# LIA-DiTella/DiffUDF

Hardware: AMD Instinct MI355X
Metric: train points/sec (SIREN fwd+∇x+Eikonal loss+bwd), 256×8 net, 100k pts (higher is better)
Workload: dtype f32

## Files before the change

### diffudf_amd/csrc/dudf_api.hip

```cpp
#include "dudf_internal.h"
#include <stdio.h>
#include <stdlib.h>
#include <string.h>
#include <vector>

namespace {
struct ProfRec { int slot; hipEvent_t e0, e1; };
bool g_prof_on = false;
std::vector<ProfRec> g_prof_recs;
std::vector<hipEvent_t> g_prof_pool;
hipEvent_t g_prof_open[PROF_NSLOTS];
const char* kProfNames[PROF_NSLOTS] = {"pack", "sweep_fwd", "sweep_rev", "sweep_adj_fwd", "sweep_adj_rev",
                                       "wgrad_hidden", "wgrad_small", "loss_fwd", "loss_bwd", "adam", "other"};
unsigned long long* g_prof_clk = nullptr;
hipEvent_t prof_event() {
    if (!g_prof_pool.empty()) { hipEvent_t e = g_prof_pool.back(); g_prof_pool.pop_back(); return e; }
    hipEvent_t e; (void)hipEventCreate(&e); return e;
}
}

namespace { int g_products[PROF_NSLOTS] = {0}; }
void dudf_note_products(int slot, int products) { if (slot >= 0 && slot < PROF_NSLOTS) g_products[slot] = products; }

unsigned long long* dudf_prof_clk(int slot) { return (g_prof_on && g_prof_clk) ? g_prof_clk + 2 * slot : nullptr; }
// ... 758 lines not shown
}

int dudf_get_option(const char* name, int* value) {
    if (!name || !value) return DUDF_E_BADMODE;
    for (int i = 0; i < OPT_COUNT; ++i)
        if (strcmp(name, kOpts[i].name) == 0) { *value = g_opt[i]; return 0; }
    return DUDF_E_BADMODE;
}

int dudf_reset_options(void) {
    for (int i = 0; i < OPT_COUNT; ++i) g_opt[i] = kOpts[i].def;
    return 0;
}

int dudf_set_wgrad_max_workgroups(int n) { return dudf_set_option("wgrad_max_workgroups", n); }

int dudf_abi_version(void) { return DUDF_ABI_VERSION; }

int dudf_profile_dump(char* buf, size_t buflen) {
    double tot[PROF_NSLOTS] = {0};
    long cnt[PROF_NSLOTS] = {0};
    for (auto& r : g_prof_recs) {
        float ms = 0.f;
        if (hipEventSynchronize(r.e1) == hipSuccess && hipEventElapsedTime(&ms, r.e0, r.e1) == hipSuccess) {
            tot[r.slot] += ms; cnt[r.slot] += 1;
        }
        g_prof_pool.push_back(r.e0); g_prof_pool.push_back(r.e1);
    }
    g_prof_recs.clear();
    size_t off = 0;
    for (int i = 0; i < PROF_NSLOTS; ++i) {
        if (!cnt[i]) continue;
        int w = snprintf(buf + off, off < buflen ? buflen - off : 0, "%s %ld %.6f\n", kProfNames[i], cnt[i], tot[i]);
        if (w < 0 || off + (size_t)w >= buflen) return DUDF_E_WORKSPACE;
        off += (size_t)w;
    }
    if (off < buflen) buf[off] = 0;
    return 0;
}

int dudf_debug_read_stash(const dudf_net_cfg* cfg, int which, int layer, int channel, int64_t n, int64_t n_hess,
                          float* out, void* workspace, size_t workspace_bytes, void* stream) {
    Ctx c;
    int rc = open_ctx(cfg, n, n_hess, workspace, workspace_bytes, stream, &c);
    if (rc) return rc;
    if (layer < 0 || layer >= c.lo.L || channel < 0 || channel > 3) return DUDF_E_BADCFG;
    const DudfLayout& lo = c.lo;
    const int64_t offs[8] = {lo.ws_S, lo.ws_C, lo.ws_Q, lo.ws_E, lo.ws_A, lo.ws_Z, lo.ws_R, lo.ws_ZS};
    if (which < 0 || which > 7) return DUDF_E_BADMODE;
    const bool sqaz = which == 0 || which == 2 || which == 4 || which == 5;
    const int b24 = which == 7 ? 0 : which == 1 ? ((lo.p24 & 4) ? 2 : 0) : sqaz ? ((lo.p24 & 1) ? 3 : 0) : ((lo.p24 & 2) ? 1 : 0);
    const int fxi = which == 0 ? 0 : which == 2 ? 1 : which == 4 ? 2 : 3;
    return dudf_launch_read_stash(lo, c.ws + offs[which], layer, channel, out, c.st, which == 1, b24,
                                  b24 == 3 ? c.ws + lo.ws_fx[fxi] : nullptr);
}

int dudf_debug_stash_layout(const dudf_net_cfg* cfg, int64_t n, int64_t n_hess, int64_t* out) {
    DudfLayout lo;
    int rc = dudf_make_layout(cfg, n, n_hess, &lo);
    if (rc) return rc;
    if (!out) return DUDF_E_BADCFG;
    const int64_t offs[8] = {lo.ws_S, lo.ws_C, lo.ws_Q, lo.ws_E, lo.ws_A, lo.ws_Z, lo.ws_R, lo.ws_ZS};
    for (int i = 0; i < 8; ++i) out[i] = offs[i] * (int64_t)sizeof(float);
    out[8] = lo.np * 16;
    out[9] = lo.stash_layer * (int64_t)sizeof(float);
    return 0;
}

int dudf_debug_kernel_choice(const dudf_net_cfg* cfg, int64_t n, int64_t n_hess, int which, int flags, char* name, size_t name_len) {
    DudfLayout lo;
    int rc = dudf_make_layout(cfg, n, n_hess, &lo, (flags & 16) != 0);
    if (rc) return rc;
    if (!name || name_len == 0) return DUDF_E_BADCFG;
    name[0] = 0;
    SweepChoice c;
    if (which == DUDF_CHOICE_WGRAD) {
        c = dudf_choose_wgrad(WgradRequest{lo.H, lo.L, lo.p24 & 1, lo.np}, dudf_options());
    } else {
        const SweepRequest r = {which & 15, lo.H, lo.L, flags & 1, (flags >> 1) & 1, (flags >> 2) & 1, (flags >> 3) & 1, split_mask(), lo.p24,
                                lo.ws_ebound != lo.ws_amax, lo.ws_zbound != lo.ws_amax};
        c = (which & DUDF_CHOICE_PAIR) ? dudf_choose_pair(r, dudf_options()) : dudf_choose_sweep(r, dudf_options());
    }
    if (c.status == 0 && dudf_choice_name(c, name, name_len) >= (int)name_len) return DUDF_E_WORKSPACE;
    return c.status;
}

int dudf_stash_mode(const dudf_net_cfg* cfg, int64_t n, int64_t n_hess) {
    DudfLayout lo;
    if (dudf_make_layout(cfg, n, n_hess, &lo)) return -1;
    return lo.p24;
}

}
```

### diffudf_amd/csrc/dudf_variants.h

```cpp
#pragma once
#include <stddef.h>
#include <stdint.h>
#include <stdio.h>
#include <utility>
#include "../../include/dudf_hip.h"

enum { SWEEP_FWD = 0, SWEEP_REV = 1, SWEEP_ADJ_FWD = 2, SWEEP_ADJ_REV = 3,
       SWEEP_FWD_H = 4, SWEEP_REV_H = 5, SWEEP_ADJ_FWD_H = 6, SWEEP_ADJ_REV_H = 7,
       SWEEP_FWD_J = 8 };

struct DudfOptions {
    int deterministic, split, split_quads, sweep_family, stash, wgrad_family, wgrad_tr, pair_launch, wgrad_max_workgroups, wgrad_buffers;
};
inline int dudf_split_mask(const DudfOptions& o) { return o.split ? (15 | (o.split_quads ? 32 : 0)) : 0; }

struct DudfVariant { int sw, fl, p24; };
constexpr DudfVariant kF32Variants[] = {{0, 3, 0}, {1, 1, 0}, {1, 0, 0}, {2, 0, 0}, {3, 1, 0}, {3, 0, 0},
                                        {4, 1, 0}, {5, 1, 0}, {5, 0, 0}, {6, 0, 0}, {7, 0, 0}, {8, 0, 0}};
constexpr DudfVariant kSweepVariants[] = {{0, 3, 1}, {0, 2, 0}, {0, 0, 0}, {1, 1, 1}, {1, 0, 0}, {2, 0, 1}, {3, 1, 1}, {3, 0, 1},
                                          {4, 1, 1}, {4, 0, 0}, {5, 1, 1}, {5, 0, 0}, {6, 0, 1}, {7, 0, 1}, {8, 0, 0}};
constexpr DudfVariant kWideVariants[] = {{0, 3, 1}, {0, 1, 0}, {1, 1, 1}, {1, 0, 0}, {2, 0, 1}, {3, 1, 1}, {3, 0, 1},
                                         {4, 1, 1}, {5, 1, 1}, {5, 0, 0}, {6, 0, 1}, {7, 0, 1}, {8, 0, 0}};
constexpr DudfVariant kPairVariants[] = {{0, 3, 1}, {1, 1, 1}, {2, 0, 1}, {3, 1, 1}};
constexpr int dudf_pair_flq(int sw) { return sw <= SWEEP_REV ? 1 : 0; }
// ... 104 lines not shown
    const bool h16 = which <= SWEEP_ADJ_REV ? ((r.split >> which) & 1) != 0 : (r.split & 32) != 0;
    int fl = fl_of(r);
    if (which == SWEEP_FWD) fl = r.store_c ? 3 : 1;
    if (which == SWEEP_FWD_H) fl = 1;
    const size_t lds16 = 3 * dudf_wide_chunk_bytes(2) + kAmaxBytes, lds = 3 * dudf_wide_chunk_bytes(3) + kAmaxBytes;
    if (r.p24) {
        const bool train_variant = which == SWEEP_FWD ? (r.store_s && r.store_c) : which == SWEEP_FWD_H ? r.store_s != 0
                                 : (which == SWEEP_REV || which == SWEEP_REV_H) ? r.train != 0 : which != SWEEP_FWD_J;
        if (r.p24 != 6 || !h16 || !train_variant) return dudf_no_choice(DUDF_E_UNSUPPORTED);
        return sweep_choice(r, DUDF_FAM_W16R, which, fl, 3, lds16, lds16);
    }
    return h16 ? sweep_choice(r, DUDF_FAM_W16, which, fl, 3, lds16, lds16) : sweep_choice(r, DUDF_FAM_W, which, fl, 6, lds, lds);
}
}

inline bool dudf_sweep_bf16_supported(int which, int H, int L) {
    return (H == 512 || H == 256 || H == 128) && L >= 2 && which >= SWEEP_FWD && which <= SWEEP_FWD_J;
}

inline SweepChoice dudf_choose_sweep(SweepRequest r, const DudfOptions& o) {
    if (r.which < SWEEP_FWD || r.which > SWEEP_FWD_J) return dudf_no_choice(DUDF_E_BADMODE);
    if (o.sweep_family && dudf_sweep_bf16_supported(r.which, r.H, r.L)) {
        const SweepChoice c = r.H == 512 ? dudf_detail::choose_w(r) : dudf_detail::choose_b(r);
        if (r.which >= SWEEP_FWD_H || c.status != DUDF_E_UNSUPPORTED) return c;
    }
    if (r.which <= SWEEP_ADJ_REV && r.p24) return dudf_no_choice(DUDF_E_UNSUPPORTED);
    if (r.which == SWEEP_FWD) r.store_s = r.store_c = 1;
    if (r.which == SWEEP_FWD_H) r.store_s = 1;
    if (!(r.H == 32 || r.H == 64 || r.H == 128 || r.H == 256 || r.H == 512)) return dudf_no_choice(DUDF_E_BADCFG);
    const int fl = r.which == SWEEP_FWD ? 3 : dudf_detail::fl_of(r);
    const size_t lds = 2 * 32 * (size_t)(r.H + 4) * sizeof(float);
    return dudf_detail::sweep_choice(r, DUDF_FAM_F32, r.which, fl, 1, lds, lds);
}

inline SweepChoice dudf_choose_pair(const SweepRequest& r, const DudfOptions& o) {
    const int base = r.which;
    const SweepChoice no = dudf_no_choice(DUDF_E_UNSUPPORTED);
    if (!o.sweep_family || !o.pair_launch || r.H != 256 || base < SWEEP_FWD || base > SWEEP_ADJ_REV) return no;
    if (!((r.split >> base) & 1) || r.L < 2 || r.L > kMaxLdsBiasLayers) return no;
    if (base == SWEEP_FWD && !(r.store_s && r.store_c)) return no;
    if (base == SWEEP_REV && !r.train) return no;
    if (base == SWEEP_ADJ_REV && !(r.have_e && r.ebound && ((r.split >> SWEEP_ADJ_FWD) & 1))) return no;
    const size_t w3 = 3 * dudf_chunk_bytes(256, 2), bias = base == SWEEP_FWD ? dudf_bias_bytes(r.L, 256) : 0;
    const size_t lds_p = w3 + (base == SWEEP_FWD ? bias : kAmaxBytes) + kOctBytes;
    const bool q16 = (r.split & 32) && r.zbound && r.ebound;
    const size_t lds_q = q16 ? w3 + bias + kAmaxBytes : 3 * dudf_chunk_bytes(256, 3) + kAmaxBytes;
    if (r.p24 && !(q16 && (r.p24 == 6 || r.p24 == 7))) return no;
    SweepChoice c = dudf_detail::sweep_choice(r, DUDF_FAM_PAIR, base, base == SWEEP_ADJ_FWD ? 0 : base == SWEEP_FWD ? 3 : 1, 3,
                                              lds_q > lds_p ? lds_q : lds_p, kLdsCu);
    c.swq = base + 4; c.flq = dudf_pair_flq(base); c.spq = q16; c.p24 = r.p24; c.no_pk = 1;
    return c;
}

struct WgradRequest { int H, L, p24; int64_t np; };
inline SweepChoice dudf_choose_wgrad(const WgradRequest& r, const DudfOptions& o) {
    const int H = r.H == 512 ? 256 : r.H, ntz = (r.H / H) * (r.H / H);
    auto pick = [&](int family, int var, int products, size_t lds) {
        SweepChoice c = {};
        c.family = family; c.H = H; c.fl = var; c.products = products; c.lds = c.lds_max = lds; c.p24 = family == DUDF_FAM_WG_F16P24;
        c.no_pk = family >= DUDF_FAM_WG_BF16P;
        return c;
    };
    if (!(H == 32 || H == 64 || H == 128 || H == 256)) return dudf_no_choice(DUDF_E_BADCFG);
    if (r.p24 && (o.wgrad_family != 0 || H != 256)) return dudf_no_choice(DUDF_E_UNSUPPORTED);
    if (o.wgrad_family == 1) return pick(DUDF_FAM_WG_F32, 0, 1, 4 * (size_t)(H / 4) * 33 * 4 * sizeof(float));
    const size_t lds_wave = (size_t)4 * 2 * (H / 4) * 16 * 4 * sizeof(float);
    if (H != 256 || o.wgrad_family == 2 || (int64_t)(r.H / 4) * r.np * 16 >= (1ll << 32)) return pick(DUDF_FAM_WG_BF16, 0, 6, lds_wave);
    const bool f16 = o.split && r.L <= kMaxAmaxLayers;
    const size_t lds_t = (size_t)(2 * 2 * 16 * 576);
    if (r.p24) {
        if (!(f16 && ntz == 1)) return dudf_no_choice(DUDF_E_UNSUPPORTED);
        return o.wgrad_buffers == 4 ? pick(DUDF_FAM_WG_F16P24, 25, 3, 4 * lds_t + 512) : pick(DUDF_FAM_WG_F16P24, 9, 3, 3 * lds_t + 512);
    }
    if (o.wgrad_tr && f16 && ntz == 1 && !o.deterministic) return pick(DUDF_FAM_WG_F16TR, 9, 3, 3 * lds_t + 512);
    const size_t lds_piece = (size_t)2 * (H / 32) * 2 * (32 * 16 + 16);
    if (f16) {
        SweepChoice c = pick(DUDF_FAM_WG_F16P, 9, 3, 3 * 2 * lds_piece + 512);
        c.remap = ntz == 4 && !o.deterministic;
        return c;
    }
    return pick(DUDF_FAM_WG_BF16P, 9, 6, 3 * 3 * lds_piece + 512);
}

inline int dudf_stash_p24_enabled(int H, int L, const DudfOptions& o) {
    int want = o.stash & 7;
    if (want != 0 && want != 6 && want != 7) want = 6;
    if (!(o.sweep_family && o.split && (dudf_split_mask(o) & 47) == 47)) want = 0;
    if (o.wgrad_family != 0) want &= 6;
    if (H == 256 && L >= 2 && L <= 32) return want;
    if (H == 512 && L >= 2) return want & 6;
    return 0;
}

inline int dudf_choice_name(const SweepChoice& c, char* buf, size_t n) {
    const char* np = c.no_pk ? "_np" : "";
    switch (c.family) {
        case DUDF_FAM_F32: return snprintf(buf, n, "sweep_kernel<%d,%d,%d>", c.H, c.sw, c.fl);
        case DUDF_FAM_BF16: return snprintf(buf, n, "sweep_bf16%s_kernel<%d,%d,%d>", np, c.H, c.sw, c.fl);
        case DUDF_FAM_F16:
            return snprintf(buf, n, "sweep_f16%s_kernel<%d,%d,%d>", np, c.H, c.sw, c.fl);
        case DUDF_FAM_F16R: return snprintf(buf, n, "sweep_f16r%s_kernel<%d,%d,%d>", np, c.H, c.sw, c.fl);
        case DUDF_FAM_F16P: return snprintf(buf, n, "sweep_f16p%s_kernel<%d,%d,%d>", np, c.H, c.sw, c.fl);
        case DUDF_FAM_W: return snprintf(buf, n, "sweep_w_kernel<%d,%d>", c.sw, c.fl);
        case DUDF_FAM_W16: return snprintf(buf, n, "sweep_w16_kernel<%d,%d>", c.sw, c.fl);
        case DUDF_FAM_W16R: return snprintf(buf, n, "sweep_w16r_kernel<%d,%d>", c.sw, c.fl);
        case DUDF_FAM_PAIR: return snprintf(buf, n, "sweep_pair_kernel<256,%d,%d,%d,%d,%d,%d>", c.swq, c.flq, c.sw, c.fl, c.spq, c.p24);
        case DUDF_FAM_WG_F32: return snprintf(buf, n, "wgrad_hidden_kernel<%d>", c.H);
        case DUDF_FAM_WG_BF16: return snprintf(buf, n, "wgrad_hidden_bf16_kernel<%d>", c.H);
        case DUDF_FAM_WG_BF16P: return snprintf(buf, n, "wgrad_hidden_bf16p_kernel<%d,%d>", c.H, c.fl);
        case DUDF_FAM_WG_F16P: return snprintf(buf, n, "wgrad_hidden_f16p_kernel<%d,%d>", c.H, c.fl);
        case DUDF_FAM_WG_F16TR: return snprintf(buf, n, "wgrad_hidden_f16tr_kernel<%d,%d>", c.H, c.fl);
        case DUDF_FAM_WG_F16P24: return snprintf(buf, n, "wgrad_hidden_f16p24_kernel<%d,%d>", c.H, c.fl);
        default: return snprintf(buf, n, "?");
    }
}
```

### diffudf_amd/csrc/dudf_wgrad.hip

```cpp
#include "dudf_internal.h"
#include <stdlib.h>
#include <string.h>
#include <type_traits>

namespace {

template <int H> struct WG;
template <> struct WG<256> { static constexpr int WO = 4, WI = 2, MT = 2, NTL = 4; };
template <> struct WG<128> { static constexpr int WO = 4, WI = 2, MT = 1, NTL = 2; };
template <> struct WG<64>  { static constexpr int WO = 2, WI = 2, MT = 1, NTL = 1; };
template <> struct WG<32>  { static constexpr int WO = 1, WI = 1, MT = 1, NTL = 1; };

constexpr int KT = 32;
constexpr int KTP = 33;

struct WgradArgs {
    const float *Q, *A, *Z, *S;
    int64_t ncol_h;
    float* dtheta;
    int64_t np, stash_layer, off_hid, hid_stride;
    int steps_total;
    int L;
    int have_g;
    int j0, nj;
    int Hs;
    int remap_nsplit;
    unsigned long long* clk;
    const unsigned* amax;
    int p24;
    const float *fxS, *fxQ, *fxA, *fxZ;
};

__device__ __forceinline__ f32x16 mfma32(float a, float b, f32x16 c) {
    return __builtin_amdgcn_mfma_f32_32x32x2f32(a, b, c, 0, 0, 0);
}

template <int H>
__device__ __forceinline__ void wgrad_hidden_body(const WgradArgs& a) {
    using W = WG<H>;
    constexpr int NTHR = 64 * W::WO * W::WI;
    constexpr int FQ = H / 4;
    constexpr int TILE = FQ * KTP * 4;
    constexpr int F4 = FQ * KT;
    constexpr int NLD = (F4 + NTHR - 1) / NTHR;
    extern __shared__ __attribute__((aligned(16))) float lds[];

    const int tid = threadIdx.x, lane = tid & 63, wave = tid >> 6;
    const int wo = wave / W::WI, wi = wave % W::WI;
    const int l32 = lane & 31, hh = lane >> 5;
    const int j = blockIdx.x + a.j0;
    const int nsplit = gridDim.y;
    const int s0 = (int)((int64_t)a.steps_total * blockIdx.y / nsplit);
    const int s1 = (int)((int64_t)a.steps_total * (blockIdx.y + 1) / nsplit);
    const int tz = a.Hs / H;
    const int o_off = (blockIdx.z / tz) * H, i_off = (blockIdx.z % tz) * H;
    const int64_t xrow = (int64_t)(o_off / 4) * a.np * 4, yrow = (int64_t)(i_off / 4) * a.np * 4;

    f32x16 acc[W::MT][W::NTL];
    float bsum[W::MT];
#pragma unroll
    for (int m = 0; m < W::MT; ++m) {
#pragma unroll
        for (int n = 0; n < W::NTL; ++n)
#pragma unroll
            for (int e = 0; e < 16; ++e) acc[m][n][e] = 0.f;
        bsum[m] = 0.f;
    }

    const int64_t lstride = a.stash_layer;
    const float* X0 = a.Q + (int64_t)(j + 1) * lstride + xrow;
    const float* X1 = a.Z + (int64_t)(j + 1) * lstride + xrow;
    const float* Y0 = a.A + (int64_t)j * lstride + yrow;
    const float* Y1 = a.S + (int64_t)j * lstride + yrow;

    f32x4 rx[NLD], ry[NLD];
    auto issue = [&](int pair, int step) {
#pragma unroll
        for (int u = 0; u < NLD; ++u) {
            const int f = tid + NTHR * u;
            if (F4 % NTHR == 0 || f < F4) {
                const int fq = f / KT, pt = f % KT;
                const int64_t off = ((int64_t)fq * a.np + (int64_t)step * KT + pt) * 4;
                rx[u] = *reinterpret_cast<const f32x4*>((pair ? X1 : X0) + off);
                ry[u] = *reinterpret_cast<const f32x4*>((pair ? Y1 : Y0) + off);
            }
        }
    };
    auto commit = [&](float* buf) {
#pragma unroll
        for (int u = 0; u < NLD; ++u) {
            const int f = tid + NTHR * u;
            if (F4 % NTHR == 0 || f < F4) {
                const int fq = f / KT, pt = f % KT;
                *reinterpret_cast<f32x4*>(buf + (fq * KTP + pt) * 4) = rx[u];
                *reinterpret_cast<f32x4*>(buf + TILE + (fq * KTP + pt) * 4) = ry[u];
            }
        }
    };

    const int npair = a.have_g ? 2 : 1;
    const int nit = npair * (s1 - s0);
    auto pair_of = [&](int it) { return a.have_g ? (it & 1) : 1; };
    auto step_of = [&](int it) { return s0 + (a.have_g ? (it >> 1) : it); };
    if (nit > 0) {
        issue(pair_of(0), step_of(0));
        commit(lds);
    }
    __syncthreads();
    for (int it = 0; it < nit; ++it) {
        const float* buf = lds + (it & 1) * 2 * TILE;
        if (it + 1 < nit) issue(pair_of(it + 1), step_of(it + 1));
        const float bflag = (pair_of(it) == 1 && wi == 0 && i_off == 0) ? 1.f : 0.f;
        const bool hstage = (int64_t)step_of(it) * KT < a.ncol_h;
        const float f_even = hstage ? (hh == 0 ? bflag : 0.f) : bflag;
// ... 610 lines not shown
        }
        DUDF_WSTAMP(4);
        if constexpr (HOT) {
            if constexpr (!(DBG & 1)) wait_raw(r, std::integral_constant<int, 2 * kSetLoads>{});
            DUDF_WSTAMP(6);
            if constexpr (!(DBG & 8)) split_store(it + 2, r, BW);
            DUDF_WSTAMP(8);
            if constexpr (!(DBG & 1)) load_raw(it + 5, r);
            publish(flag0 + 4u * (unsigned)wave, (unsigned)it + 3u);
        } else if (it + 2 < nit) {
            split_store(it + 2, r, BW);
            if (it + 5 < nit) load_raw_plain(it + 5, r);
            publish(flag0 + 4u * (unsigned)wave, (unsigned)it + 3u);
        }
        DUDF_WSTAMP(10);
        DUDF_WSTAMP(11);
    };
    int it = 0;
    const int nhot = nit >= 8 ? ((nit - 5) / 3) * 3 : 0;
    auto drain = [&]() {
        asm volatile("s_waitcnt vmcnt(0)" : "+v"(R0.g0), "+v"(R0.g1), "+v"(R0.g2), "+v"(R0.g3), "+v"(R1.g0), "+v"(R1.g1),
                     "+v"(R1.g2), "+v"(R1.g3), "+v"(R2.g0), "+v"(R2.g1), "+v"(R2.g2), "+v"(R2.g3));
        if constexpr (P24 == 1) asm volatile("" : "+v"(R0.sc), "+v"(R1.sc), "+v"(R2.sc));
    };
    drain();
    using B0 = std::integral_constant<int, 0>; using B1 = std::integral_constant<int, 1>; using B2 = std::integral_constant<int, 2>;
    for (; it < nhot; it += 3) {
        stage(it, R2, std::true_type{}, B0{});
        stage(it + 1, R0, std::true_type{}, B1{});
        stage(it + 2, R1, std::true_type{}, B2{});
    }
    drain();
    for (; it < nit; it += 3) {
        stage(it, R2, std::false_type{}, B0{});
        if (it + 1 < nit) stage(it + 1, R0, std::false_type{}, B1{});
        if (it + 2 < nit) stage(it + 2, R1, std::false_type{}, B2{});
    }
#if DUDF_WGRAD_DBG & 32
    if (bx == 3 && by == 10 && lane == 0)
        for (int i = 0; i < 12; ++i) g_wstamp[wave][i] = wst[i];
#endif

    float* dW = a.dtheta + a.off_hid + (int64_t)j * a.hid_stride + (int64_t)o_off * a.Hs + i_off;
    float* dB = a.dtheta + a.off_hid + (int64_t)j * a.hid_stride + (int64_t)a.Hs * a.Hs + o_off;
    if (nit > 0) {
        const int l32 = lane & 31, hh = lane >> 5;
#pragma unroll
        for (int m = 0; m < W::MT; ++m)
#pragma unroll
            for (int e = 0; e < 16; ++e) {
                const int o = (wo * W::MT + m) * 32 + (e & 3) + 8 * (e >> 2) + 4 * hh;
#pragma unroll
                for (int n = 0; n < W::NTL; ++n) {
                    const int i = (wi * W::NTL + n) * 32 + l32;
#if DUDF_WGRAD_DBG & 64
                    asm volatile("" :: "v"(acc[m][n][e]));
#else
                    atomicAdd(dW + (int64_t)o * a.Hs + i, SP != 0 ? acc[m][n][e] * inv_p : acc[m][n][e]);
#endif
                }
            }
        if (p_oper == 0 && i_off == 0) {
            if constexpr (P24 != 0) {
                const float bun = P24 == 1 ? 1.0f / sc1 : 1.0f;
                auto red = [&](float v, int f) {
                    v += __shfl_xor(v, 1); v += __shfl_xor(v, 2); v += __shfl_xor(v, 4); v += __shfl_xor(v, 8);
                    if (p_li == 0) atomicAdd(dB + f, v * bun);
                };
                const f32x4 bs[4] = {bacc, bacc1, bacc2, bacc3};
#pragma unroll
                for (int t = 0; t < 4; ++t)
#pragma unroll
                    for (int e = 0; e < 4; ++e) red(bs[t][e], 16 * (4 * pw + t) + 4 * p_q + e);
            } else {
            auto red = [&](float v, int f) {
                v += __shfl_xor(v, 1);
                v += __shfl_xor(v, 2);
                if (p_cg == 0) atomicAdd(dB + 4 * p_fq + f, v);
            };
            red(bacc.x, 0); red(bacc.y, 1); red(bacc.z, 2); red(bacc.w, 3);
            }
        }
    }
    if (clk_on && tid == 0) {
        a.clk[0] = __builtin_amdgcn_s_memtime() - clk_t0;
        a.clk[1] = __builtin_amdgcn_s_memrealtime() - clk_r0;
    }
}
template <int VAR> constexpr int wg_buffers() { static_assert(VAR == 9 || VAR == 25, "VAR 9: three image buffers, 25: four"); return VAR == 25 ? 4 : 3; }
template <int H, int VAR>
__global__ __launch_bounds__(64 * WG<H>::WO * WG<H>::WI) DUDF_NO_PK void wgrad_hidden_bf16p_kernel(WgradArgs a) {
    wgrad_hidden_bf16p_body<H, wg_buffers<VAR>()>(a);
}
template <int H, int VAR>
__global__ __launch_bounds__(64 * WG<H>::WO * WG<H>::WI) DUDF_NO_PK void wgrad_hidden_f16p_kernel(WgradArgs a) {
    wgrad_hidden_bf16p_body<H, wg_buffers<VAR>(), 1>(a);
}
template <int H, int VAR>
__global__ __launch_bounds__(64 * WG<H>::WO * WG<H>::WI) DUDF_NO_PK void wgrad_hidden_f16tr_kernel(WgradArgs a) {
    wgrad_hidden_bf16p_body<H, wg_buffers<VAR>(), 1, 2>(a);
}
template <int H, int VAR>
__global__ __launch_bounds__(64 * WG<H>::WO * WG<H>::WI) DUDF_NO_PK void wgrad_hidden_f16p24_kernel(WgradArgs a) {
    wgrad_hidden_bf16p_body<H, wg_buffers<VAR>(), 1, 1>(a);
}

#ifndef DUDF_WGSMALL_P24_PTS
#define DUDF_WGSMALL_P24_PTS 4096
#endif
struct WgradSmallArgs {
    const float *Q, *A, *Z, *S;
    const float *x4, *gbar, *ybar;
    float* dtheta;
    int64_t np, ncols, stash_layer, off_wo, off_bo;
    int H, L, have_g;
    int pts_per_block;
    float rho;
    const float *fxS, *fxQ, *fxA, *fxZ;
};

__device__ __forceinline__ float wave_sum(float v) {
#pragma unroll
    for (int o = 32; o > 0; o >>= 1) v += __shfl_xor(v, o);
    return v;
}

__device__ __forceinline__ void wgrad_small_body(const WgradSmallArgs& a) {
    const int lane = threadIdx.x & 63, wave = threadIdx.x >> 6;
    const int FQ = a.H / 4;
    const int64_t p0 = (int64_t)blockIdx.x * a.pts_per_block;
    const int64_t p1 = (p0 + a.pts_per_block < a.ncols) ? p0 + a.pts_per_block : a.ncols;
    const float* Q0 = a.Q;
    const float* Z0 = a.Z;
    const float* AL = a.A + (int64_t)(a.L - 1) * a.stash_layer;
    const float* SL = a.S + (int64_t)(a.L - 1) * a.stash_layer;
    const int fq_per = (FQ + gridDim.y - 1) / gridDim.y;
    const int fq_lo = blockIdx.y * fq_per, fq_hi = (fq_lo + fq_per < FQ) ? fq_lo + fq_per : FQ;
    for (int fq = fq_lo + wave; fq < fq_hi; fq += 4) {
        float w1[4][4], wo[4];
#pragma unroll
        for (int c = 0; c < 4; ++c) { wo[c] = 0.f; w1[c][0] = w1[c][1] = w1[c][2] = w1[c][3] = 0.f; }
#pragma unroll 4
        for (int64_t p = p0 + lane; p < p1; p += 64) {
            const int64_t off = ((int64_t)fq * a.np + p) * 4;
            const f32x4 z = __builtin_nontemporal_load(reinterpret_cast<const f32x4*>(Z0 + off));
            const f32x4 sl = __builtin_nontemporal_load(reinterpret_cast<const f32x4*>(SL + off));
            const f32x4 xv = *reinterpret_cast<const f32x4*>(a.x4 + p * 4);
            const float yb = a.ybar[p];
            f32x4 qv = {0, 0, 0, 0}, al = {0, 0, 0, 0}, gb = {0, 0, 0, 0};
            if (a.have_g) {
                qv = __builtin_nontemporal_load(reinterpret_cast<const f32x4*>(Q0 + off));
                al = __builtin_nontemporal_load(reinterpret_cast<const f32x4*>(AL + off));
                gb = *reinterpret_cast<const f32x4*>(a.gbar + p * 4);
            }
#pragma unroll
            for (int c = 0; c < 4; ++c) {
#pragma unroll
                for (int d = 0; d < 4; ++d) w1[c][d] += qv[c] * gb[d] + z[c] * xv[d];
                wo[c] += al[c] * xv[3] + yb * sl[c];
            }
        }
#pragma unroll
        for (int c = 0; c < 4; ++c) {
            const int f = 4 * fq + c;
#pragma unroll
            for (int d = 0; d < 4; ++d) {
                const float v = wave_sum(w1[c][d]);
                if (lane == 0) atomicAdd(d < 3 ? a.dtheta + f * 3 + d : a.dtheta + 3 * a.H + f, a.rho * v);
            }
            const float vo = wave_sum(wo[c]);
            if (lane == 0) atomicAdd(a.dtheta + a.off_wo + f, vo);
        }
    }
    if (wave == 0 && blockIdx.y == 0) {
        float s = 0.f;
        for (int64_t p = p0 + lane; p < p1; p += 64) s += a.ybar[p];
        s = wave_sum(s);
        if (lane == 0) atomicAdd(a.dtheta + a.off_bo, s);
    }
}
__global__ __launch_bounds__(256) DUDF_NO_PK void wgrad_small_kernel(WgradSmallArgs a) { wgrad_small_body(a); }

__device__ __forceinline__ f32x4 small_unpack24(const unsigned* g, const float sc) {
    typedef unsigned u3_t __attribute__((ext_vector_type(3)));
    const u3_t d = __builtin_nontemporal_load(reinterpret_cast<const u3_t*>(g));
    const unsigned d0 = d.x, d1 = d.y, d2 = d.z;
    const unsigned m = 0x00ffffffu, two = 0x40000000u;
    const unsigned y = __builtin_amdgcn_perm(d1, d0, 0x0c0c0703u);
    const unsigned t3 = __builtin_amdgcn_perm(d2, y, 0x0c070100u) | two;
    const float m3 = -3.0f * sc;
    return f32x4{__builtin_fmaf(__uint_as_float((d0 & m) | two), sc, m3), __builtin_fmaf(__uint_as_float((d1 & m) | two), sc, m3),
                 __builtin_fmaf(__uint_as_float((d2 & m) | two), sc, m3), __builtin_fmaf(__uint_as_float(t3), sc, m3)};
}
__global__ __launch_bounds__(256) DUDF_NO_PK void wgrad_small_p24_kernel(WgradSmallArgs a) {
    const int lane = threadIdx.x & 63, wave = threadIdx.x >> 6;
    const int q = lane >> 4, li = lane & 15, T = blockIdx.y;
    const int64_t ng = a.np >> 4;
    const int64_t g0 = (int64_t)blockIdx.x * (a.pts_per_block >> 4);
    const int64_t gend = (a.ncols + 15) >> 4;
    const int64_t g1 = g0 + (a.pts_per_block >> 4) < gend ? g0 + (a.pts_per_block >> 4) : gend;
    const int64_t lbytes = a.stash_layer * 3;
    auto tile = [&](const float* arr, int layer) { return reinterpret_cast<const char*>(arr) + (int64_t)layer * lbytes + (int64_t)T * ng * 768 + lane * 12; };
    const char* Q0 = tile(a.Q, 0); const char* Z0 = tile(a.Z, 0);
    const char* AL = tile(a.A, a.L - 1); const char* SL = tile(a.S, a.L - 1);
    float w1[4][4], wo[4];
#pragma unroll
    for (int c = 0; c < 4; ++c) { wo[c] = 0.f; w1[c][0] = w1[c][1] = w1[c][2] = w1[c][3] = 0.f; }
    float sy = 0.f;
    const int nwave = (int)(blockDim.x >> 6);
#pragma unroll 4
    for (int64_t g = g0 + wave; g < g1; g += nwave) {
        const int64_t p = g * 16 + li;
        const f32x4 z = small_unpack24(reinterpret_cast<const unsigned*>(Z0 + g * 768), a.fxZ[p]);
        const f32x4 sl = small_unpack24(reinterpret_cast<const unsigned*>(SL + g * 768), a.fxS[(int64_t)(a.L - 1) * a.np + p]);
        const f32x4 xv = *reinterpret_cast<const f32x4*>(a.x4 + p * 4);
        const float yb = a.ybar[p];
        f32x4 qv = {0, 0, 0, 0}, al = {0, 0, 0, 0}, gb = {0, 0, 0, 0};
        if (a.have_g) {
            qv = small_unpack24(reinterpret_cast<const unsigned*>(Q0 + g * 768), a.fxQ[p]);
            al = small_unpack24(reinterpret_cast<const unsigned*>(AL + g * 768), a.fxA[(int64_t)(a.L - 1) * a.np + p]);
            gb = *reinterpret_cast<const f32x4*>(a.gbar + p * 4);
        }
        sy += yb;
#pragma unroll
        for (int c = 0; c < 4; ++c) {
#pragma unroll
            for (int d = 0; d < 4; ++d) w1[c][d] += qv[c] * gb[d] + z[c] * xv[d];
            wo[c] += al[c] * xv[3] + yb * sl[c];
        }
    }
    auto sum16 = [](float v) { v += __shfl_xor(v, 1); v += __shfl_xor(v, 2); v += __shfl_xor(v, 4); v += __shfl_xor(v, 8); return v; };
    __shared__ float red[4][4][21];
#pragma unroll
    for (int c = 0; c < 4; ++c) {
#pragma unroll
        for (int d = 0; d < 4; ++d) {
            const float v = sum16(w1[c][d]);
            if (li == 0) red[wave][q][c * 4 + d] = v;
        }
        const float vo = sum16(wo[c]);
        if (li == 0) red[wave][q][16 + c] = vo;
    }
    {
        const float v = sum16(sy);
        if (li == 0) red[wave][q][20] = v;
    }
    __syncthreads();
    for (int t = threadIdx.x; t < 81; t += blockDim.x) {
        if (t < 80) {
            const int qq = t / 20, k = t % 20;
            float v = 0.f;
            for (int w = 0; w < nwave; ++w) v += red[w][qq][k];
            if (k < 16) {
                const int c = k >> 2, d = k & 3, f = 16 * T + 4 * qq + c;
                atomicAdd(d < 3 ? a.dtheta + f * 3 + d : a.dtheta + 3 * a.H + f, a.rho * v);
            } else {
                atomicAdd(a.dtheta + a.off_wo + 16 * T + 4 * qq + (k - 16), v);
            }
        } else if (T == 0) {
            float v = 0.f;
            for (int w = 0; w < nwave; ++w) v += red[w][0][20];
            atomicAdd(a.dtheta + a.off_bo, v);
        }
    }
}

static_assert(KTP == 33 && NRING == 4 && KB == 16, "dudf_choose_wgrad: LDS sizes");
template <int H>
int launch_hidden(const SweepChoice& c, const WgradArgs& a, hipStream_t st) {
    using W = WG<H>;
    const int tz = a.Hs / H, ntz = tz * tz;
    int nsplit = dudf_wgrad_max_workgroups() / (a.nj * ntz);
    if (nsplit > a.steps_total) nsplit = a.steps_total;
    if (nsplit < 1 || dudf_deterministic()) nsplit = 1;
    const dim3 grid(a.nj, nsplit, ntz), block(64 * W::WO * W::WI);
    if (c.family == DUDF_FAM_WG_F32) return dudf_launch_kernel<&wgrad_hidden_kernel<H>>(grid, block, c.lds, c.lds_max, st, a);
    if (c.family == DUDF_FAM_WG_BF16) return dudf_launch_kernel<&wgrad_hidden_bf16_kernel<H>>(grid, block, c.lds, c.lds_max, st, a);
    if constexpr (H == 256) {
        if (c.family == DUDF_FAM_WG_F16P24 && c.fl == 25) return dudf_launch_kernel<&wgrad_hidden_f16p24_kernel<H, 25>>(grid, block, c.lds, c.lds_max, st, a);
        if (c.family == DUDF_FAM_WG_F16P24) return dudf_launch_kernel<&wgrad_hidden_f16p24_kernel<H, 9>>(grid, block, c.lds, c.lds_max, st, a);
        if (c.family == DUDF_FAM_WG_F16TR) return dudf_launch_kernel<&wgrad_hidden_f16tr_kernel<H, 9>>(grid, block, c.lds, c.lds_max, st, a);
        if (c.family == DUDF_FAM_WG_BF16P) return dudf_launch_kernel<&wgrad_hidden_bf16p_kernel<H, 9>>(grid, block, c.lds, c.lds_max, st, a);
        if (c.family == DUDF_FAM_WG_F16P && c.remap) {
            WgradArgs b = a;
            b.remap_nsplit = nsplit;
            return dudf_launch_kernel<&wgrad_hidden_f16p_kernel<H, 9>>(dim3(((a.nj * nsplit + 7) / 8) * 32), block, c.lds, c.lds_max, st, b);
        }
        if (c.family == DUDF_FAM_WG_F16P) return dudf_launch_kernel<&wgrad_hidden_f16p_kernel<H, 9>>(grid, block, c.lds, c.lds_max, st, a);
    }
    return DUDF_E_UNSUPPORTED;
}

}

int dudf_launch_wgrad(const DudfLayout& lo, float* ws, float* dtheta, int have_g, hipStream_t st, int layer_begin,
                      int layer_end) {
    if (layer_begin < 0) layer_begin = 0;
    if (layer_end > lo.L + 1) layer_end = lo.L + 1;
    WgradArgs a;
    a.Q = ws + lo.ws_Q; a.A = ws + lo.ws_A; a.Z = ws + lo.ws_Z; a.S = ws + lo.ws_S; a.ncol_h = lo.ncol_h;
    a.dtheta = dtheta; a.np = lo.np; a.stash_layer = lo.stash_layer;
    a.off_hid = lo.off_hid; a.hid_stride = lo.hid_stride; a.steps_total = (int)(lo.ncols / KT); a.L = lo.L;
    a.have_g = have_g; a.Hs = lo.H;
    a.amax = reinterpret_cast<const unsigned*>(ws + lo.ws_amax);
    a.clk = dudf_prof_clk(PROF_WGRAD_HIDDEN);
    a.remap_nsplit = 0;
    a.p24 = lo.p24 & 1;
    a.fxS = ws + lo.ws_fx[0]; a.fxQ = ws + lo.ws_fx[1]; a.fxA = ws + lo.ws_fx[2]; a.fxZ = ws + lo.ws_fx[3];
    const int hb = layer_begin < 1 ? 1 : layer_begin, he = layer_end > lo.L ? lo.L : layer_end;
    a.j0 = hb - 1; a.nj = he > hb ? he - hb : 0;
    int rc = 0;
    if (a.nj > 0) {
        DudfProfScope prof(PROF_WGRAD_HIDDEN, st);
        const SweepChoice c = dudf_choose_wgrad(WgradRequest{lo.H, lo.L, a.p24, lo.np}, dudf_options());
        if (c.status) return c.status;
        dudf_note_products(PROF_WGRAD_HIDDEN, c.products);
        switch (c.H) {
            case 32: rc = launch_hidden<32>(c, a, st); break;
            case 64: rc = launch_hidden<64>(c, a, st); break;
            case 128: rc = launch_hidden<128>(c, a, st); break;
            default: rc = launch_hidden<256>(c, a, st); break;
        }
    }
    if (rc) return rc;
    if (!(layer_begin <= 0 || layer_end >= lo.L + 1)) return 0;
    WgradSmallArgs s;
    s.Q = a.Q; s.A = a.A; s.Z = a.Z; s.S = a.S; s.x4 = ws + lo.ws_x4; s.gbar = ws + lo.ws_gbar; s.ybar = ws + lo.ws_ybar;
    s.dtheta = dtheta; s.np = lo.np; s.ncols = lo.ncols; s.stash_layer = lo.stash_layer;
    s.off_wo = lo.off_wo; s.off_bo = lo.off_bo; s.H = lo.H; s.L = lo.L; s.have_g = have_g; s.rho = lo.rho;
    s.fxS = a.fxS; s.fxQ = a.fxQ; s.fxA = a.fxA; s.fxZ = a.fxZ;
    s.pts_per_block = dudf_deterministic() ? (int)lo.ncols : 4096;
    const int grid = (int)((lo.ncols + s.pts_per_block - 1) / s.pts_per_block);
    DudfProfScope prof(PROF_WGRAD_SMALL, st);
    const int fqn = lo.H / 4;
    const int gy = fqn >= 64 ? 16 : (fqn >= 4 ? fqn / 4 : 1);
    if (lo.p24 & 1) {
        if (!dudf_deterministic()) {
            s.pts_per_block = DUDF_WGSMALL_P24_PTS;
            const int64_t want = (lo.ncols / 30 + 255) / 256 * 256;
            if (want < s.pts_per_block) s.pts_per_block = want < 512 ? 512 : (int)want;
        }
        s.pts_per_block = (s.pts_per_block + 15) / 16 * 16;
        hipLaunchKernelGGL(wgrad_small_p24_kernel, dim3((unsigned)((lo.ncols + s.pts_per_block - 1) / s.pts_per_block), lo.H / 16),
                           dim3(dudf_deterministic() ? 64 : 256), 0, st, s);
        return (int)hipGetLastError();
    }
    hipLaunchKernelGGL(wgrad_small_kernel, dim3(grid, gy), dim3(256), 0, st, s);
    return (int)hipGetLastError();
}
```

### include/dudf_hip.h

```cpp
#ifndef DUDF_HIP_H
#define DUDF_HIP_H
#include <stddef.h>
#include <stdint.h>

#ifdef __cplusplus
extern "C" {
#endif

#define DUDF_ABI_VERSION 8
int dudf_abi_version(void);

#define DUDF_E_BADCFG   (-1)
#define DUDF_E_WORKSPACE (-2)
#define DUDF_E_BADMODE  (-3)
#define DUDF_E_UNSUPPORTED (-4)

#define DUDF_LOSS_S1    0
#define DUDF_LOSS_S2    1
#define DUDF_LOSS_SIREN 2

typedef struct dudf_net_cfg {
    int32_t n_in;
    int32_t n_hidden_layers;
    int32_t hidden;
// ... 62 lines not shown
#define DUDF_SHADE_PHONG 0
#define DUDF_SHADE_WARD  1
int dudf_render_shade(int model, const unsigned char* hits, int64_t m, const int32_t* rows, int64_t k, const double* hit_pos,
                      const double* normals, const double* pc1, const double* pc2, const double* color_map, const double* light_position,
                      const double* camera_position, double shininess, double alpha1, double alpha2, double* accumulator, void* stream);

int dudf_render_finish(const double* accumulator, int64_t count, double sample_rate, unsigned char* out_image, void* stream);

size_t dudf_nearest_workspace_bytes(int64_t n);
int dudf_nearest_points(const float* x, int64_t n, const float* y, int64_t m, int norm, float* out_dist, int64_t* out_idx,
                        void* workspace, size_t workspace_bytes, void* stream);

size_t dudf_chamfer_terms_workspace_bytes(int64_t n);
int dudf_chamfer_terms(const float* dist, const int64_t* idx, int64_t n, const float* x_normals, const float* y_normals, int64_t m,
                       double* out_sums, void* workspace, size_t workspace_bytes, void* stream);

size_t dudf_vertex_normals_workspace_bytes(int64_t n_vertices);
int dudf_vertex_normals(const double* vertices, int64_t n_vertices, const int64_t* faces, int64_t n_faces, float* out_normals,
                        void* workspace, size_t workspace_bytes, void* stream);

#define DUDF_MESH_INDEX_FLAGS_OFFSET 24
#define DUDF_MESH_FLAG_NONFINITE 1
#define DUDF_MESH_FLAG_BAD_ORDER 2
size_t dudf_mesh_index_bytes(int64_t n_tri);
int dudf_mesh_morton_codes(const float* tri, int64_t n_tri, void* index, size_t index_bytes, int64_t* codes, void* stream);
int dudf_mesh_index_build(const float* tri, int64_t n_tri, const int64_t* order, void* index, size_t index_bytes, void* stream);
int dudf_mesh_distance(const float* tri, int64_t n_tri, const void* index, size_t index_bytes, const float* pts, int64_t n_pts,
                       float* out_dist, int64_t* out_tri, float* out_closest, int64_t* out_stats, void* stream);

int dudf_grid_fields(const dudf_net_cfg* cfg, const float* theta, int64_t grid_n, int64_t start, int64_t count,
                     int inverse_mode, double alpha, float* out_df, float* out_vec, int* out_flag_count,
                     void* workspace, size_t workspace_bytes, void* stream);

size_t dudf_capudf_workspace_bytes(int64_t grid_n);
int dudf_capudf_count(const float* ndf, const float* grad, int64_t grid_n, double threshold, int64_t* out_counts,
                      void* workspace, size_t workspace_bytes, void* stream);
int dudf_capudf_emit(const float* ndf, const float* grad, int64_t grid_n, double threshold, double* out_vertices,
                     int64_t* out_triangles, int64_t* out_cells, void* workspace, size_t workspace_bytes, void* stream);

int dudf_loss_forward(const dudf_net_cfg* cfg, int mode, const float* theta,
                      const float* x, const float* normals, const float* sdf,
                      int64_t n_local, int64_t n_global, int64_t n_hess, const double* weights, double alpha,
                      float* out_terms, void* workspace, size_t workspace_bytes, void* stream);

int dudf_s2_forward_stats(const dudf_net_cfg* cfg, const float* theta, const float* x, const float* sdf,
                          int64_t n_local, double* stats, void* workspace, size_t workspace_bytes,
                          void* stream);
int dudf_s2_terms(const double* stats, const double* weights, float* out_terms, void* stream);

int dudf_loss_backward(const dudf_net_cfg* cfg, int mode, const float* theta,
                       const float* x, const float* normals, const float* sdf,
                       int64_t n_local, int64_t n_global, int64_t n_hess, const double* weights, double alpha,
                       const float* cot, const double* stats, float* dtheta, int accumulate,
                       void* workspace, size_t workspace_bytes, void* stream);

int dudf_loss_backward_sweeps(const dudf_net_cfg* cfg, int mode, const float* theta, const float* normals, const float* sdf,
                              int64_t n_local, int64_t n_global, int64_t n_hess, const double* weights, double alpha,
                              const float* cot, const double* stats, void* workspace, size_t workspace_bytes, void* stream);
int dudf_weight_gradient(const dudf_net_cfg* cfg, int64_t n_local, int64_t n_hess, int have_gradient_terms, int layer_begin,
                         int layer_end, float* dtheta, int accumulate, void* workspace, size_t workspace_bytes, void* stream);

int dudf_fields_forward(const dudf_net_cfg* cfg, const float* theta, const float* x, int64_t n,
                        float* out_f, float* out_g, void* workspace, size_t workspace_bytes, void* stream);
int dudf_fields_backward(const dudf_net_cfg* cfg, const float* theta, const float* x, int64_t n,
                         const float* ybar, const float* gbar, float* dtheta, int accumulate,
                         void* workspace, size_t workspace_bytes, void* stream);

int dudf_adam_step(float* theta, const float* dtheta, float* exp_avg, float* exp_avg_sq, int64_t n,
                   double lr, double beta1, double beta2, double eps, int64_t step, double grad_scale,
                   void* stream);

int dudf_adam_schedule(const double* lr, int64_t n_steps, int64_t first_step, double beta1, double beta2, float* out);
int dudf_adam_step_scheduled(float* theta, const float* dtheta, float* exp_avg, float* exp_avg_sq, int64_t n,
                             double beta1, double beta2, double eps, const float* sched, int64_t n_rows, const int64_t* row,
                             double grad_scale, void* stream);

int dudf_debug_read_stash(const dudf_net_cfg* cfg, int which, int layer, int channel, int64_t n, int64_t n_hess,
                          float* out, void* workspace, size_t workspace_bytes, void* stream);

int dudf_debug_stash_layout(const dudf_net_cfg* cfg, int64_t n, int64_t n_hess, int64_t* out);

#define DUDF_CHOICE_PAIR 16
#define DUDF_CHOICE_WGRAD (-1)
int dudf_debug_kernel_choice(const dudf_net_cfg* cfg, int64_t n, int64_t n_hess, int which, int flags, char* name, size_t name_len);

int dudf_stash_mode(const dudf_net_cfg* cfg, int64_t n, int64_t n_hess);

int dudf_sample_batch(const float* tri, int64_t n_tri, const float* pc_pos, const float* pc_nrm, int64_t n_pc,
                      int64_t n_on, int64_t n_far, int64_t n_near, uint64_t seed, uint64_t step, int rank, int world,
                      float* x, float* normals, float* sdf, void* stream);
int dudf_sample_batch_at(const float* tri, int64_t n_tri, const float* pc_pos, const float* pc_nrm, int64_t n_pc,
                         int64_t n_on, int64_t n_far, int64_t n_near, uint64_t seed, const int64_t* step_dev, int rank, int world,
                         float* x, float* normals, float* sdf, void* stream);

int dudf_profile_enable(int on);
int dudf_profile_dump(char* buf, size_t buflen);
int dudf_profile_clocks(char* buf, size_t buflen);
int dudf_profile_products(char* buf, size_t buflen);

int dudf_set_option(const char* name, int value);
int dudf_get_option(const char* name, int* value);
int dudf_reset_options(void);
int dudf_set_wgrad_max_workgroups(int n);

const char* dudf_version(void);
int dudf_split_mode(void);

int dudf_sweeps_bf16x6(const dudf_net_cfg* cfg);

#ifdef __cplusplus
}
#endif
#endif
```

Measured before the change: 38.77 million.

## Fuse thin-layer weight gradient into tail of p24 hidden wgrad kernel

Folds the first/last-layer (thin) weight-gradient reduction into the epilogue of the f16 p24 hidden-layer wgrad kernel. The work is spread evenly across all hidden-kernel workgroups, and the separate small-layer launch is skipped when the fused path is on. The aim is to drop one kernel launch and its tail/idle cost. In exchange, the hidden kernel takes a second kernel argument that it reads through the raw kernarg pointer, and every workgroup does an extra barrier-separated reduction loop that may lengthen its critical path.

```diff
diff --git a/diffudf_amd/csrc/dudf_api.hip b/diffudf_amd/csrc/dudf_api.hip
--- a/diffudf_amd/csrc/dudf_api.hip
+++ b/diffudf_amd/csrc/dudf_api.hip
@@ -864,6 +864,12 @@
         c = (which & DUDF_CHOICE_PAIR) ? dudf_choose_pair(r, dudf_options()) : dudf_choose_sweep(r, dudf_options());
     }
     if (c.status == 0 && dudf_choice_name(c, name, name_len) >= (int)name_len) return DUDF_E_WORKSPACE;
+    if (c.status == 0 && which == DUDF_CHOICE_WGRAD && (flags & DUDF_CHOICE_ALL_LAYERS) &&
+        dudf_wgrad_thin_epilogue(c, lo.L, 0, lo.L + 1, dudf_options())) {
+        const size_t len = strlen(name);
+        if (len + sizeof(DUDF_CHOICE_THIN_SUFFIX) > name_len) return DUDF_E_WORKSPACE;
+        memcpy(name + len, DUDF_CHOICE_THIN_SUFFIX, sizeof(DUDF_CHOICE_THIN_SUFFIX));
+    }
     return c.status;
 }
 
diff --git a/diffudf_amd/csrc/dudf_variants.h b/diffudf_amd/csrc/dudf_variants.h
--- a/diffudf_amd/csrc/dudf_variants.h
+++ b/diffudf_amd/csrc/dudf_variants.h
@@ -210,6 +210,10 @@
     return pick(DUDF_FAM_WG_BF16P, 9, 6, 3 * 3 * lds_piece + 512);
 }
 
+inline bool dudf_wgrad_thin_epilogue(const SweepChoice& c, int L, int layer_begin, int layer_end, const DudfOptions& o) {
+    return c.status == 0 && c.family == DUDF_FAM_WG_F16P24 && L >= 2 && layer_begin <= 0 && layer_end >= L + 1 && !o.deterministic;
+}
+
 inline int dudf_stash_p24_enabled(int H, int L, const DudfOptions& o) {
     int want = o.stash & 7;
     if (want != 0 && want != 6 && want != 7) want = 6;
diff --git a/diffudf_amd/csrc/dudf_wgrad.hip b/diffudf_amd/csrc/dudf_wgrad.hip
--- a/diffudf_amd/csrc/dudf_wgrad.hip
+++ b/diffudf_amd/csrc/dudf_wgrad.hip
@@ -13,6 +13,22 @@
 
 constexpr int KT = 32;
 constexpr int KTP = 33;
+
+#ifndef DUDF_WGSMALL_P24_PTS
+#define DUDF_WGSMALL_P24_PTS 4096
+#endif
+struct WgradSmallArgs {
+    const float *Q, *A, *Z, *S;
+    const float *x4, *gbar, *ybar;
+    float* dtheta;
+    int64_t np, ncols, stash_layer, off_wo, off_bo;
+    int H, L, have_g;
+    int pts_per_block;
+    float rho;
+    const float *fxS, *fxQ, *fxA, *fxZ;
+};
+template <bool ROW16>
+__device__ __forceinline__ void wgrad_small_p24_share(const WgradSmallArgs& a, float* red, int T, int64_t g0, int64_t g1, int lane, int wave, int nwave);
 
 struct WgradArgs {
     const float *Q, *A, *Z, *S;
@@ -30,6 +46,7 @@
     int p24;
     const float *fxS, *fxQ, *fxA, *fxZ;
 };
+struct WgradThinArgs { int on; WgradSmallArgs sm; };
 
 __device__ __forceinline__ f32x16 mfma32(float a, float b, f32x16 c) {
     return __builtin_amdgcn_mfma_f32_32x32x2f32(a, b, c, 0, 0, 0);
@@ -806,6 +823,25 @@
             }
         }
     }
+    if constexpr (P24 == 1) {
+        static_assert(alignof(WgradThinArgs) == 8 && sizeof(WgradArgs) % 8 == 0, "offset of the second kernel argument");
+        const __attribute__((address_space(4))) char* kp = (const __attribute__((address_space(4))) char*)__builtin_amdgcn_kernarg_segment_ptr();
+        asm volatile("" : "+s"(kp));
+        const WgradThinArgs* thin = (const WgradThinArgs*)(kp + sizeof(WgradArgs));
+        if (thin->on) {
+            const int elane = (int)__builtin_amdgcn_mbcnt_hi(~0u, __builtin_amdgcn_mbcnt_lo(~0u, 0u));
+            const int64_t nwg = (int64_t)gridDim.x * gridDim.y, w = (int64_t)by * gridDim.x + bx;
+            const int64_t G = (thin->sm.ncols + 15) >> 4, U = 16 * G;
+            const int64_t u1 = U * (w + 1) / nwg;
+            for (int64_t u = U * w / nwg; u < u1;) {
+                const int T = (int)(u / G);
+                const int64_t g0 = u - T * G, g1 = g0 + (u1 - u) < G ? g0 + (u1 - u) : G;
+                __syncthreads();
+                wgrad_small_p24_share<false>(thin->sm, reinterpret_cast<float*>(ldsb), T, g0, g1, elane, wave, NW_);
+                u += g1 - g0;
+            }
+        }
+    }
     if (clk_on && tid == 0) {
         a.clk[0] = __builtin_amdgcn_s_memtime() - clk_t0;
         a.clk[1] = __builtin_amdgcn_s_memrealtime() - clk_r0;
@@ -825,23 +861,9 @@
     wgrad_hidden_bf16p_body<H, wg_buffers<VAR>(), 1, 2>(a);
 }
 template <int H, int VAR>
-__global__ __launch_bounds__(64 * WG<H>::WO * WG<H>::WI) DUDF_NO_PK void wgrad_hidden_f16p24_kernel(WgradArgs a) {
+__global__ __launch_bounds__(64 * WG<H>::WO * WG<H>::WI) DUDF_NO_PK void wgrad_hidden_f16p24_kernel(WgradArgs a, WgradThinArgs) {
     wgrad_hidden_bf16p_body<H, wg_buffers<VAR>(), 1, 1>(a);
 }
-
-#ifndef DUDF_WGSMALL_P24_PTS
-#define DUDF_WGSMALL_P24_PTS 4096
-#endif
-struct WgradSmallArgs {
-    const float *Q, *A, *Z, *S;
-    const float *x4, *gbar, *ybar;
-    float* dtheta;
-    int64_t np, ncols, stash_layer, off_wo, off_bo;
-    int H, L, have_g;
-    int pts_per_block;
-    float rho;
-    const float *fxS, *fxQ, *fxA, *fxZ;
-};
 
 __device__ __forceinline__ float wave_sum(float v) {
 #pragma unroll
@@ -916,13 +938,21 @@
     return f32x4{__builtin_fmaf(__uint_as_float((d0 & m) | two), sc, m3), __builtin_fmaf(__uint_as_float((d1 & m) | two), sc, m3),
                  __builtin_fmaf(__uint_as_float((d2 & m) | two), sc, m3), __builtin_fmaf(__uint_as_float(t3), sc, m3)};
 }
-__global__ __launch_bounds__(256) DUDF_NO_PK void wgrad_small_p24_kernel(WgradSmallArgs a) {
-    const int lane = threadIdx.x & 63, wave = threadIdx.x >> 6;
-    const int q = lane >> 4, li = lane & 15, T = blockIdx.y;
+template <bool ROW16>
+__device__ __forceinline__ f32x4 small_row4(const float* p) {
+    if constexpr (ROW16) {
+        return *reinterpret_cast<const f32x4*>(p);
+    } else {
+        const float* hi = p + 2;
+        asm volatile("" : "+v"(hi));
+        const f32x2 u = *reinterpret_cast<const f32x2*>(p), v = *reinterpret_cast<const f32x2*>(hi);
+        return f32x4{u.x, u.y, v.x, v.y};
+    }
+}
+template <bool ROW16>
+__device__ __forceinline__ void wgrad_small_p24_share(const WgradSmallArgs& a, float* red, int T, int64_t g0, int64_t g1, int lane, int wave, int nwave) {
+    const int q = lane >> 4, li = lane & 15;
     const int64_t ng = a.np >> 4;
-    const int64_t g0 = (int64_t)blockIdx.x * (a.pts_per_block >> 4);
-    const int64_t gend = (a.ncols + 15) >> 4;
-    const int64_t g1 = g0 + (a.pts_per_block >> 4) < gend ? g0 + (a.pts_per_block >> 4) : gend;
     const int64_t lbytes = a.stash_layer * 3;
     auto tile = [&](const float* arr, int layer) { return reinterpret_cast<const char*>(arr) + (int64_t)layer * lbytes + (int64_t)T * ng * 768 + lane * 12; };
     const char* Q0 = tile(a.Q, 0); const char* Z0 = tile(a.Z, 0);
@@ -931,19 +961,18 @@
 #pragma unroll
     for (int c = 0; c < 4; ++c) { wo[c] = 0.f; w1[c][0] = w1[c][1] = w1[c][2] = w1[c][3] = 0.f; }
     float sy = 0.f;
-    const int nwave = (int)(blockDim.x >> 6);
 #pragma unroll 4
     for (int64_t g = g0 + wave; g < g1; g += nwave) {
         const int64_t p = g * 16 + li;
         const f32x4 z = small_unpack24(reinterpret_cast<const unsigned*>(Z0 + g * 768), a.fxZ[p]);
         const f32x4 sl = small_unpack24(reinterpret_cast<const unsigned*>(SL + g * 768), a.fxS[(int64_t)(a.L - 1) * a.np + p]);
-        const f32x4 xv = *reinterpret_cast<const f32x4*>(a.x4 + p * 4);
+        const f32x4 xv = small_row4<ROW16>(a.x4 + p * 4);
         const float yb = a.ybar[p];
         f32x4 qv = {0, 0, 0, 0}, al = {0, 0, 0, 0}, gb = {0, 0, 0, 0};
         if (a.have_g) {
             qv = small_unpack24(reinterpret_cast<const unsigned*>(Q0 + g * 768), a.fxQ[p]);
             al = small_unpack24(reinterpret_cast<const unsigned*>(AL + g * 768), a.fxA[(int64_t)(a.L - 1) * a.np + p]);
-            gb = *reinterpret_cast<const f32x4*>(a.gbar + p * 4);
+            gb = small_row4<ROW16>(a.gbar + p * 4);
         }
         sy += yb;
 #pragma unroll
@@ -954,27 +983,27 @@
         }
     }
     auto sum16 = [](float v) { v += __shfl_xor(v, 1); v += __shfl_xor(v, 2); v += __shfl_xor(v, 4); v += __shfl_xor(v, 8); return v; };
-    __shared__ float red[4][4][21];
+    float* mine = red + (wave * 4 + q) * 21;
 #pragma unroll
     for (int c = 0; c < 4; ++c) {
 #pragma unroll
         for (int d = 0; d < 4; ++d) {
             const float v = sum16(w1[c][d]);
-            if (li == 0) red[wave][q][c * 4 + d] = v;
+            if (li == 0) mine[c * 4 + d] = v;
         }
         const float vo = sum16(wo[c]);
-        if (li == 0) red[wave][q][16 + c] = vo;
+        if (li == 0) mine[16 + c] = vo;
     }
     {
         const float v = sum16(sy);
-        if (li == 0) red[wave][q][20] = v;
+        if (li == 0) mine[20] = v;
     }
     __syncthreads();
-    for (int t = threadIdx.x; t < 81; t += blockDim.x) {
+    for (int t = wave * 64 + lane; t < 81; t += nwave * 64) {
         if (t < 80) {
             const int qq = t / 20, k = t % 20;
             float v = 0.f;
-            for (int w = 0; w < nwave; ++w) v += red[w][qq][k];
+            for (int w = 0; w < nwave; ++w) v += red[(w * 4 + qq) * 21 + k];
             if (k < 16) {
                 const int c = k >> 2, d = k & 3, f = 16 * T + 4 * qq + c;
                 atomicAdd(d < 3 ? a.dtheta + f * 3 + d : a.dtheta + 3 * a.H + f, a.rho * v);
@@ -983,15 +1012,22 @@
             }
         } else if (T == 0) {
             float v = 0.f;
-            for (int w = 0; w < nwave; ++w) v += red[w][0][20];
+            for (int w = 0; w < nwave; ++w) v += red[(w * 4) * 21 + 20];
             atomicAdd(a.dtheta + a.off_bo, v);
         }
     }
+}
+__global__ __launch_bounds__(256) DUDF_NO_PK void wgrad_small_p24_kernel(WgradSmallArgs a) {
+    __shared__ float red[4 * 4 * 21];
+    const int64_t g0 = (int64_t)blockIdx.x * (a.pts_per_block >> 4);
+    const int64_t gend = (a.ncols + 15) >> 4;
+    const int64_t g1 = g0 + (a.pts_per_block >> 4) < gend ? g0 + (a.pts_per_block >> 4) : gend;
+    wgrad_small_p24_share<true>(a, red, blockIdx.y, g0, g1, threadIdx.x & 63, threadIdx.x >> 6, (int)(blockDim.x >> 6));
 }
 
 static_assert(KTP == 33 && NRING == 4 && KB == 16, "dudf_choose_wgrad: LDS sizes");
 template <int H>
-int launch_hidden(const SweepChoice& c, const WgradArgs& a, hipStream_t st) {
+int launch_hidden(const SweepChoice& c, const WgradArgs& a, const WgradThinArgs& thin, hipStream_t st) {
     using W = WG<H>;
     const int tz = a.Hs / H, ntz = tz * tz;
     int nsplit = dudf_wgrad_max_workgroups() / (a.nj * ntz);
@@ -1001,8 +1037,8 @@
     if (c.family == DUDF_FAM_WG_F32) return dudf_launch_kernel<&wgrad_hidden_kernel<H>>(grid, block, c.lds, c.lds_max, st, a);
     if (c.family == DUDF_FAM_WG_BF16) return dudf_launch_kernel<&wgrad_hidden_bf16_kernel<H>>(grid, block, c.lds, c.lds_max, st, a);
     if constexpr (H == 256) {
-        if (c.family == DUDF_FAM_WG_F16P24 && c.fl == 25) return dudf_launch_kernel<&wgrad_hidden_f16p24_kernel<H, 25>>(grid, block, c.lds, c.lds_max, st, a);
-        if (c.family == DUDF_FAM_WG_F16P24) return dudf_launch_kernel<&wgrad_hidden_f16p24_kernel<H, 9>>(grid, block, c.lds, c.lds_max, st, a);
+        if (c.family == DUDF_FAM_WG_F16P24 && c.fl == 25) return dudf_launch_kernel<&wgrad_hidden_f16p24_kernel<H, 25>>(grid, block, c.lds, c.lds_max, st, a, thin);
+        if (c.family == DUDF_FAM_WG_F16P24) return dudf_launch_kernel<&wgrad_hidden_f16p24_kernel<H, 9>>(grid, block, c.lds, c.lds_max, st, a, thin);
         if (c.family == DUDF_FAM_WG_F16TR) return dudf_launch_kernel<&wgrad_hidden_f16tr_kernel<H, 9>>(grid, block, c.lds, c.lds_max, st, a);
         if (c.family == DUDF_FAM_WG_BF16P) return dudf_launch_kernel<&wgrad_hidden_bf16p_kernel<H, 9>>(grid, block, c.lds, c.lds_max, st, a);
         if (c.family == DUDF_FAM_WG_F16P && c.remap) {
@@ -1033,26 +1069,29 @@
     a.fxS = ws + lo.ws_fx[0]; a.fxQ = ws + lo.ws_fx[1]; a.fxA = ws + lo.ws_fx[2]; a.fxZ = ws + lo.ws_fx[3];
     const int hb = layer_begin < 1 ? 1 : layer_begin, he = layer_end > lo.L ? lo.L : layer_end;
     a.j0 = hb - 1; a.nj = he > hb ? he - hb : 0;
+    WgradSmallArgs s;
+    s.Q = a.Q; s.A = a.A; s.Z = a.Z; s.S = a.S; s.x4 = ws + lo.ws_x4; s.gbar = ws + lo.ws_gbar; s.ybar = ws + lo.ws_ybar;
+    s.dtheta = dtheta; s.np = lo.np; s.ncols = lo.ncols; s.stash_layer = lo.stash_layer;
+    s.off_wo = lo.off_wo; s.off_bo = lo.off_bo; s.H = lo.H; s.L = lo.L; s.have_g = have_g; s.rho = lo.rho;
+    s.fxS = a.fxS; s.fxQ = a.fxQ; s.fxA = a.fxA; s.fxZ = a.fxZ;
+    s.pts_per_block = 0;
+    WgradThinArgs thin = {0, s};
     int rc = 0;
     if (a.nj > 0) {
         DudfProfScope prof(PROF_WGRAD_HIDDEN, st);
         const SweepChoice c = dudf_choose_wgrad(WgradRequest{lo.H, lo.L, a.p24, lo.np}, dudf_options());
         if (c.status) return c.status;
+        thin.on = dudf_wgrad_thin_epilogue(c, lo.L, layer_begin, layer_end, dudf_options()) ? 1 : 0;
         dudf_note_products(PROF_WGRAD_HIDDEN, c.products);
         switch (c.H) {
-            case 32: rc = launch_hidden<32>(c, a, st); break;
-            case 64: rc = launch_hidden<64>(c, a, st); break;
-            case 128: rc = launch_hidden<128>(c, a, st); break;
-            default: rc = launch_hidden<256>(c, a, st); break;
-        }
-    }
-    if (rc) return rc;
+            case 32: rc = launch_hidden<32>(c, a, thin, st); break;
+            case 64: rc = launch_hidden<64>(c, a, thin, st); break;
+            case 128: rc = launch_hidden<128>(c, a, thin, st); break;
+            default: rc = launch_hidden<256>(c, a, thin, st); break;
+        }
+    }
+    if (rc || thin.on) return rc;
     if (!(layer_begin <= 0 || layer_end >= lo.L + 1)) return 0;
-    WgradSmallArgs s;
-    s.Q = a.Q; s.A = a.A; s.Z = a.Z; s.S = a.S; s.x4 = ws + lo.ws_x4; s.gbar = ws + lo.ws_gbar; s.ybar = ws + lo.ws_ybar;
-    s.dtheta = dtheta; s.np = lo.np; s.ncols = lo.ncols; s.stash_layer = lo.stash_layer;
-    s.off_wo = lo.off_wo; s.off_bo = lo.off_bo; s.H = lo.H; s.L = lo.L; s.have_g = have_g; s.rho = lo.rho;
-    s.fxS = a.fxS; s.fxQ = a.fxQ; s.fxA = a.fxA; s.fxZ = a.fxZ;
     s.pts_per_block = dudf_deterministic() ? (int)lo.ncols : 4096;
     const int grid = (int)((lo.ncols + s.pts_per_block - 1) / s.pts_per_block);
     DudfProfScope prof(PROF_WGRAD_SMALL, st);
diff --git a/include/dudf_hip.h b/include/dudf_hip.h
--- a/include/dudf_hip.h
+++ b/include/dudf_hip.h
@@ -168,6 +168,8 @@
 
 #define DUDF_CHOICE_PAIR 16
 #define DUDF_CHOICE_WGRAD (-1)
+#define DUDF_CHOICE_ALL_LAYERS 32
+#define DUDF_CHOICE_THIN_SUFFIX "+thin"
 int dudf_debug_kernel_choice(const dudf_net_cfg* cfg, int64_t n, int64_t n_hess, int which, int flags, char* name, size_t name_len);
 
 int dudf_stash_mode(const dudf_net_cfg* cfg, int64_t n, int64_t n_hess);
```

After: 39.05 million, median of 4. About the same (+0.7%).
